# nagadomi/nunif

Measured on AMD Instinct MI355X. Metric: input MPix/s, waifu2x swin_unet 2x tiled render (tile 256) of 1080p frames, higher is better.
Workload: dtype f16; 1 GPU; waifu2x swin_unet 2x (art scale2x geometry), tile_size=256, 1080p frame, random-init weights; tile_size=256, tile_batch=45, tiles_per_frame=45, concurrent_streams=2, parallelism=frame-sharded x1

## Files before the change

### nunif_amd/csrc/swin_kernels.h

```cpp
#pragma once
#include "common.h"

namespace nunif {

struct GemmArgs {
    const f16 *a; int B, Hi, Wi, Cin;
    int Ho, Wo, stride, oy, ox, kw;
    int K;
    const f16 *w;
    const float *bias;
    int N;
    int mode;
    int act;
    float slope;
    const f16 *res;
    void *out;
    int ldo;
    int n_real;
    int ps;
    int oshift, OH, OW;
    int no_clamp;
    int lda;
    int rev;
    int nt_chunk;
    int res_H = 0, res_W = 0, res_crop = 0;
    const float *in_scale = nullptr;
};
int launch_gemm(const GemmArgs &g, hipStream_t s, const char *tag);

struct PatchUpArgs { const f16 *a, *w; const float *bias; const f16 *res; f16 *out; int B, Ho, Wo, Cq, rev; };
bool patchup_supported(const PatchUpArgs &g);
int launch_patchup(const PatchUpArgs &g, hipStream_t s);

struct PatchDownArgs { const f16 *a, *w; const float *bias; f16 *out; int B, Ho, Wo, Cin, oy, rev; int N = 192; int act = 0; float slope = 0.f; };
bool patchdown_supported(const PatchDownArgs &g);
int launch_patchdown(const PatchDownArgs &g, hipStream_t s);

struct CunetUpArgs { const f16 *a, *w; const float *bias; const f16 *res; f16 *out; const float *in_scale; int B, S, res_S, crop;
                     float slope; };
bool cunet_up_supported(const CunetUpArgs &g);
int launch_cunet_up(const CunetUpArgs &g, hipStream_t s);

struct GemmOsArgs {
    const f16 *a; long M; int lda, K;
    const f16 *w; const float *bias; int N;
    int act;
    const f16 *res;
    f16 *out; int ldo;
    float2 *stats_out;
    const float2 *stats_in; int stats_parts; const float *wsum; float ln_eps;
};
bool gemm_os_supported(long M, int N, int K);
bool gemm_os_consumes_stats(long M, int N, int K);
int launch_gemm_os(const GemmOsArgs &g, hipStream_t s, const char *tag);

struct DaMlpArgs {
    f16 *t; long M;
    const f16 *w1; const float *b1, *ws1;
    const f16 *w2c; const float *b2;
    const float2 *stats_in; float2 *stats_out; float ln_eps;
    void *partial; unsigned *flags;
};
bool da_mlp_supported(int D, int hidden);

struct CunetHeadArgs { const f16 *a, *w; const float *bias; float *out32; const float *add32; int B, Hi, Wi, Ho, Wo, addH, addW, add_crop, clamp01; };
bool cunet_head_supported(const CunetHeadArgs &g);
int launch_cunet_head(const CunetHeadArgs &g, hipStream_t s);

constexpr int kVdaGnBlocks = 256;
int launch_vda_groupnorm(const f16 *x, const float *gamma, const float *beta, f16 *y, float2 *part, int frames, int P, int C, float eps, hipStream_t s);
int launch_vda_layernorm(const f16 *x, const float *gamma, const float *beta, f16 *y, long T, int C, float eps, hipStream_t s);
int launch_vda_geglu(const f16 *h, f16 *out, long T, int I, hipStream_t s);
struct VdaTattnArgs { const f16 *qkv; f16 *kc, *vc; const float *pq, *pk, *pv; f16 *att; int P, C, hd, start, idx; };
int launch_vda_tattn(const VdaTattnArgs &g, hipStream_t s);
long da_mlp_partial_bytes(long M);
long da_mlp_flag_count(long M);
int launch_da_mlp(const DaMlpArgs &a, hipStream_t s);

struct Stem1Args {
    const float *x;
    int frame_mode, H, W, wb, istep, pad_t, pad_l, tile_begin;
    int B, T;
    const float *w;
    const float *bias;
    int C1, C1P;
    f16 *out;
    float slope;
};
int launch_stem1(const Stem1Args &a, hipStream_t s);

struct StemFusedArgs {
    const float *x;
    int frame_mode, H, W, wb, istep, pad_t, pad_l, tile_begin;
    int B, T;
    const f16 *w1;
    const f16 *w2;
    const float *b2;
    f16 *out;
    float slope;
    int rev;
    int C1, C, crop;
};
bool stem_fused_supported(int C1, int C);
int launch_stem_fused(const StemFusedArgs &a, hipStream_t s);

int proj_mlp_stream_frags(int C);
struct TailToImage { const f16 *w; const float *bias; float *out; int H, W, ps, n_real; };
struct WinMap { int on, H, W, shift; const int *pixmap; };
int launch_winmap_build(int *pixmap, int B, int H, int W, int shift, hipStream_t s);
int launch_proj_mlp(const f16 *att, f16 *x, const f16 *wstream, const float *bp, const float *b0, const float *b3,
                    long M, int C, hipStream_t s, const TailToImage *to_image = nullptr, int rev = 0,
                    const WinMap *wm = nullptr, int gelu32 = 0);

int swin_block96_tail_frags();
int swin_block96_btab_floats();
int launch_swin_block96(f16 *x, const f16 *wqkv, const float *bqkv, const float *btab, const f16 *wtail, const float *bp,
                        const float *b0, const float *b3, int B, int H, int W, int shift, hipStream_t s,
// ... 62 lines not shown
```

### nunif_amd/csrc/swin_patchdown.hip

```cpp
#include <algorithm>
#include <cstdlib>

#include "swin_kernels.h"

namespace nunif {

#define MFMA_16x16x32(a, b, c) __builtin_amdgcn_mfma_f32_16x16x32_f16((a), (b), (c), 0, 0, 0)

namespace {
constexpr int kWaves = 8;
constexpr int kMF = 2;

__device__ __forceinline__ void dma16(const void *src, unsigned lds_byte_addr) {
    asm volatile("s_mov_b32 m0, %1\n\ts_nop 0\n\tglobal_load_lds_dwordx4 %0, off" ::"v"(src), "s"(lds_byte_addr) : "memory");
}
}

template <int CIN, int kKS, int kNT, bool LRELU>
__global__ void __launch_bounds__(kWaves * 64) patchdown_kernel(PatchDownArgs g) {
    static_assert(CIN == 64 || CIN == 96 || CIN == 192, "Cin");
    constexpr int kWBytes = kNT * kKS * 1024;
    extern __shared__ __attribute__((aligned(1024))) unsigned char smem_pd[];
    const f16x8 *wres = reinterpret_cast<const f16x8 *>(smem_pd);
    const float4 *bres = reinterpret_cast<const float4 *>(smem_pd + kWBytes);
    const int tid = threadIdx.x, lane = tid & 63, r16 = lane & 15, grp = lane >> 4;
    const int wave = __builtin_amdgcn_readfirstlane(tid >> 6);
    {
        const unsigned char *src = reinterpret_cast<const unsigned char *>(g.w) + lane * 16;
        const unsigned lds0 = (unsigned)reinterpret_cast<size_t>(smem_pd);
#pragma unroll
        for (int u = 0; u < kWBytes / 1024 / kWaves; ++u) {
            const int i = wave + kWaves * u;
            dma16(src + (size_t)i * 1024, lds0 + i * 1024);
        }
        if (tid < kNT * 4) reinterpret_cast<float4 *>(smem_pd + kWBytes)[tid] = reinterpret_cast<const float4 *>(g.bias)[tid];
    }
    const unsigned Wo = (unsigned)g.Wo, Ho = (unsigned)g.Ho, Wi = 2 * Wo, Hi = 2 * Ho;
    const unsigned M = (unsigned)g.B * Ho * Wo;
    const unsigned n_groups = (M + kMF * 16 - 1) / (kMF * 16);
    const unsigned step = gridDim.x * kWaves;
    unsigned gi = blockIdx.x * kWaves + wave;
    const bool any = gi < n_groups;
    const int prc = pair_run_channel(grp);

    struct Grp { unsigned in[kMF], out[kMF]; };
    auto coords = [&](unsigned gidx, Grp &c) {
        const unsigned gg = g.rev ? n_groups - 1 - gidx : gidx;
#pragma unroll
        for (int f = 0; f < kMF; ++f) {
            unsigned m = gg * (kMF * 16) + f * 16 + r16;
            m = m < M ? m : M - 1;
            const unsigned t = m / Wo, x = m - t * Wo;
            const unsigned b = t / Ho, y = t - b * Ho;
            c.in[f] = (((b * Hi + 2 * y + (unsigned)g.oy) * Wi + 2 * x) * CIN + grp * 8) * 2;
            c.out[f] = (m * (kNT * 16) + prc) * 2;
        }
    };
    auto ks_off = [&](int ks) -> unsigned {
        const int k0 = ks * 32, tap = k0 / CIN, c0 = k0 % CIN;
        const int dy = tap / 2, dx = tap % 2;
        return (unsigned)((dy * Wi + dx) * CIN + c0) * 2;
    };
    auto load_frag = [&](const Grp &c, int f, int ks) -> f16x8 {
        const unsigned char *base = reinterpret_cast<const unsigned char *>(g.a) + (size_t)ks_off(ks);
        return *reinterpret_cast<const f16x8 *>(base + (size_t)c.in[f]);
    };

    Grp cur, nxt;
    f16x8 xf[kMF][kKS];
    coords(any ? gi : 0, cur);
#pragma unroll
    for (int ks = 0; ks < kKS; ++ks) {
#pragma unroll
        for (int f = 0; f < kMF; ++f) xf[f][ks] = load_frag(cur, f, ks);
    }
    asm volatile("s_waitcnt vmcnt(0)" ::: "memory");
#pragma unroll
    for (int ks = 0; ks < kKS; ++ks) {
#pragma unroll
        for (int f = 0; f < kMF; ++f) asm volatile("" : "+v"(xf[f][ks]));
    }
    __syncthreads();
    if (!any) return;

    while (true) {
        const unsigned gn = gi + step;
        const bool has_next = gn < n_groups;
        coords(has_next ? gn : gi, nxt);
        int lofs = lane;
        asm volatile("" : "+v"(lofs));
        f32x4 acc[kNT][kMF];
#pragma unroll
        for (int nt = 0; nt < kNT; ++nt) {
            const float4 bv = bres[nt * 4 + (lofs >> 4)];
#pragma unroll
            for (int f = 0; f < kMF; ++f) acc[nt][f] = (f32x4){bv.x, bv.y, bv.z, bv.w};
        }
#pragma unroll
        for (int ks = 0; ks < kKS; ++ks) {
#pragma unroll
            for (int nt = 0; nt < kNT; ++nt) {
                const f16x8 wv = wres[(nt * kKS + ks) * 64 + lofs];
#pragma unroll
                for (int f = 0; f < kMF; ++f) acc[nt][f] = MFMA_16x16x32(wv, xf[f][ks], acc[nt][f]);
            }
#pragma unroll
            for (int f = 0; f < kMF; ++f) xf[f][ks] = load_frag(nxt, f, ks);
            __builtin_amdgcn_sched_barrier(0);
        }
        unsigned char *obase = reinterpret_cast<unsigned char *>(g.out);
#pragma unroll
        for (int p = 0; p < kNT / 2; ++p) {
#pragma unroll
            for (int f = 0; f < kMF; ++f) {
                f32x4 a0 = acc[2 * p][f], a1 = acc[2 * p + 1][f];
                if constexpr (LRELU) {
#pragma unroll
                    for (int r = 0; r < 4; ++r) {
                        a0[r] = a0[r] >= 0.f ? a0[r] : a0[r] * g.slope;
                        a1[r] = a1[r] >= 0.f ? a1[r] : a1[r] * g.slope;
                    }
                }
                const f16x8 ov = pair_to_run((f16x4){(f16)a0[0], (f16)a0[1], (f16)a0[2], (f16)a0[3]},
                                             (f16x4){(f16)a1[0], (f16)a1[1], (f16)a1[2], (f16)a1[3]});
                *reinterpret_cast<f16x8 *>(obase + (size_t)cur.out[f] + p * 64) = ov;
            }
        }
        if (!has_next) break;
        cur = nxt;
        gi = gn;
    }
}

bool patchdown_supported(const PatchDownArgs &g) {
    if (const char *e = getenv("NUNIF_PATCHDOWN")) if (atoi(e) == 0) return false;
    const long M = (long)g.B * g.Ho * g.Wo;
    const bool shape = (g.Cin == 96 && g.N == 192 && g.oy == 0) || (g.Cin == 192 && g.N == 192 && (g.oy == 0 || g.oy == 1)) ||
                       (g.Cin == 64 && g.N == 64 && g.oy == 0);
    const bool act_ok = g.Cin == 64 ? g.act == 2 : g.act == 0;
    return shape && M > 0 && 4 * M * g.Cin * 2 < (1L << 32) && M * g.N * 2 < (1L << 32) && act_ok;
}

template <int CIN, int KS, int NT, bool LRELU>
static int launch_pd(const PatchDownArgs &g, hipStream_t s, const char *name, int wgs_per_cu) {
    constexpr int smem = NT * KS * 1024 + NT * 16 * 4;
    static_assert(smem <= 160 * 1024, "LDS");
    const long M = (long)g.B * g.Ho * g.Wo;
    static bool configured = false;
    static int cus = 256;
    if (!configured) {
        NUNIF_HIP_CHECK(hipFuncSetAttribute((const void *)patchdown_kernel<CIN, KS, NT, LRELU>, hipFuncAttributeMaxDynamicSharedMemorySize, smem));
        int dev = 0;
        NUNIF_HIP_CHECK(hipGetDevice(&dev));
        NUNIF_HIP_CHECK(hipDeviceGetAttribute(&cus, hipDeviceAttributeMultiprocessorCount, dev));
        configured = true;
    }
    const long groups = (M + kMF * 16 - 1) / (kMF * 16);
    const unsigned grid = (unsigned)std::max<long>(1, std::min<long>((groups + kWaves - 1) / kWaves, (long)cus * wgs_per_cu));
    ProfScope ps(name, s, 2.0 * (double)M * (KS * 32.0) * (NT * 16.0), (double)M * (KS * 32.0 + NT * 16.0) * 2.0);
    patchdown_kernel<CIN, KS, NT, LRELU><<<grid, kWaves * 64, smem, s>>>(g);
    NUNIF_LAUNCH_CHECK();
    return NUNIF_HIP_OK;
}

int launch_patchdown(const PatchDownArgs &g, hipStream_t s) {
    NUNIF_REQUIRE(g.a && g.w && g.bias && g.out && patchdown_supported(g), "patchdown: bad argument");
    if (g.Cin == 96) return launch_pd<96, 12, 12, false>(g, s, "patchdown_kernel<96>", 1);
    if (g.Cin == 192) return launch_pd<192, 12, 12, false>(g, s, "patchdown_kernel<192>", 1);
    return launch_pd<64, 8, 4, true>(g, s, "patchdown_kernel<64>", 2);
}

}
```

### nunif_amd/csrc/swin_stem.hip

```cpp
#include <algorithm>
#include <cstdlib>
#include <cstring>

#include "swin_kernels.h"

namespace nunif {

#define MFMA_16x16x32(a, b, c) __builtin_amdgcn_mfma_f32_16x16x32_f16((a), (b), (c), 0, 0, 0)

namespace {
constexpr int kTile = 16;
constexpr int kWaves = 8;

template <int C1, int C, int CROP, int ROWS>
struct StemGeom {
    static constexpr int kTH = kWaves * ROWS;
    static constexpr int kS1H = kTH + 2, kS1W = kTile + 2;
    static constexpr int kInH = kTH + 4, kInW = kTile + 4;
    static constexpr int kInElems = 3 * kInH * kInW;
    static constexpr int kInBytes = (kInElems + 8) * 2;
    static constexpr int kPix = C1 * 2 + 16;
    static constexpr int kKS2 = (9 * C1 + 31) / 32;
    static constexpr int kNT1 = C1 / 16, kNT2 = C / 16;
    static constexpr int kW2Bytes = kKS2 * kNT2 * 1024, kW1Bytes = kNT1 * 1024, kS1Bytes = kS1H * kS1W * kPix;
// ... 90 lines not shown
    __syncthreads();

#pragma unroll 1
    for (int t = blockIdx.x; t < n_tiles; t += gridDim.x) {
        const int tm = tmap(t);
        const int txt = tm % ntx, t2 = tm / ntx;
        const int tyt = t2 % nty, b = t2 / nty;
        f16x8 w1f[kNT1];
#pragma unroll
        for (int nt = 0; nt < kNT1; ++nt) w1f[nt] = w1g[nt * 64 + lane];
#pragma unroll
        for (int i = 0; i < kNIn; ++i) {
            const int e = tid + kWaves * 64 * i;
            if (e < kInElems) inl[e] = (f16)pin[i];
        }
        __syncthreads();
#pragma unroll
        for (int i = 0; i < kR1; ++i) {
            const int mt = wave + kWaves * i;
            if (mt * 16 < kS1H * kS1W) {
                const int p = min(mt * 16 + r16, kS1H * kS1W - 1);
                const int py = p / kS1W, px = p - py * kS1W;
                const int pb = py * kInW + px;
                f16x8 bfrag;
#pragma unroll
                for (int j = 0; j < 8; ++j) bfrag[j] = inl[ioff[j] + ((cmask >> j) & 1u ? 0 : pb)];
                const bool wr = mt * 16 + r16 < kS1H * kS1W;
#pragma unroll
                for (int nt = 0; nt < kNT1; ++nt) {
                    f32x4 acc = {0.f, 0.f, 0.f, 0.f};
                    acc = MFMA_16x16x32(w1f[nt], bfrag, acc);
                    f16x4 o;
#pragma unroll
                    for (int q = 0; q < 4; ++q) o[q] = (f16)(acc[q] >= 0.f ? acc[q] : acc[q] * a.slope);
                    if (wr) *reinterpret_cast<f16x4 *>(s1l + p * kPix + (16 * nt + 4 * grp) * 2) = o;
                }
            }
        }
        __syncthreads();
        if (t + (int)gridDim.x < n_tiles) fetch_in(tmap(t + gridDim.x), pin);
        f32x4 acc[kNT2][ROWS];
#pragma unroll
        for (int nt = 0; nt < kNT2; ++nt) {
            const f32x4 bb = *reinterpret_cast<const f32x4 *>(b2l + 16 * nt + 4 * grp);
#pragma unroll
            for (int f = 0; f < ROWS; ++f) acc[nt][f] = bb;
        }
        const unsigned char *bp0 = s1l + ((ROWS * wave) * kS1W + r16) * kPix;
#pragma unroll
        for (int ks = 0; ks < kKS2; ++ks) {
            f16x8 bf[ROWS];
#pragma unroll
            for (int f = 0; f < ROWS; ++f) bf[f] = *reinterpret_cast<const f16x8 *>(bp0 + f * (kS1W * kPix) + koff[ks]);
#pragma unroll
            for (int nt = 0; nt < kNT2; ++nt) {
                const f16x8 w = w2l[(ks * kNT2 + nt) * 64 + lane];
#pragma unroll
                for (int f = 0; f < ROWS; ++f) acc[nt][f] = MFMA_16x16x32(w, bf[f], acc[nt][f]);
            }
        }
        const int ox = kTile * txt + r16;
#pragma unroll
        for (int f = 0; f < ROWS; ++f) {
            const int oy = kTH * tyt + ROWS * wave + f;
            const bool ok = oy < S && ox < S;
            f16 *op = a.out + (((long)b * S + min(oy, S - 1)) * S + min(ox, S - 1)) * kC + pair_run_channel(grp);
#pragma unroll
            for (int p = 0; p < kNT2 / 2; ++p) {
                f16x4 oa, ob;
#pragma unroll
                for (int q = 0; q < 4; ++q) {
                    const float u = acc[2 * p][f][q], v = acc[2 * p + 1][f][q];
                    oa[q] = (f16)(u >= 0.f ? u : u * a.slope);
                    ob[q] = (f16)(v >= 0.f ? v : v * a.slope);
                }
                const f16x8 o = pair_to_run(oa, ob);
                if (ok) *reinterpret_cast<f16x8 *>(op + 32 * p) = o;
            }
        }
        __syncthreads();
    }
}

bool stem_fused_supported(int C1, int C) { return (C1 == 48 && C == 96) || (C1 == 32 && C == 64); }

template <int C1, int C, int CROP, int ROWS>
static int launch_stem_t(const StemFusedArgs &a, hipStream_t s, const char *name) {
    typedef StemGeom<C1, C, CROP, ROWS> G;
    const int S = a.T - 4 - 2 * CROP;
    NUNIF_REQUIRE(S > 0, "stem: tile size %d too small", a.T);
    const int ntx = (S + kTile - 1) / kTile, nty = (S + G::kTH - 1) / G::kTH;
    const long n_tiles = (long)a.B * ntx * nty;
    if (n_tiles == 0) return NUNIF_HIP_OK;
    const double px = (double)a.B * S * S;
    ProfScope ps(name, s, 2.0 * px * (27.0 * C1 + 9.0 * C1 * C), px * (12.0 + C * 2.0));
    static bool configured = false;
    if (!configured) {
        NUNIF_HIP_CHECK(hipFuncSetAttribute((const void *)stem_fused_kernel<C1, C, CROP, ROWS>, hipFuncAttributeMaxDynamicSharedMemorySize,
                                            G::kSmem));
        configured = true;
    }
    const unsigned grid = (unsigned)std::min<long>(n_tiles, G::kSmem <= 80 * 1024 ? 512 : 256);
    stem_fused_kernel<C1, C, CROP, ROWS><<<grid, kWaves * 64, G::kSmem, s>>>(a);
    NUNIF_LAUNCH_CHECK();
    return NUNIF_HIP_OK;
}

int launch_stem_fused(const StemFusedArgs &a, hipStream_t s) {
    static const int rows = getenv("NUNIF_STEM_ROWS") && atoi(getenv("NUNIF_STEM_ROWS")) == 2 ? 2 : 3;
    static const int rows_c = getenv("NUNIF_STEM_ROWS_CUNET") && atoi(getenv("NUNIF_STEM_ROWS_CUNET")) == 3 ? 3 : 2;
    if (a.C1 == 32 && a.C == 64 && a.crop == 0)
        return rows_c == 3 ? launch_stem_t<32, 64, 0, 3>(a, s, "stem_fused_kernel<32,64>") : launch_stem_t<32, 64, 0, 2>(a, s, "stem_fused_kernel<32,64>");
    NUNIF_REQUIRE((a.C1 == 48 || a.C1 == 0) && (a.C == 96 || a.C == 0), "stem: C1=%d C=%d unsupported", a.C1, a.C);
    return rows == 3 ? launch_stem_t<48, 96, 6, 3>(a, s, "stem_fused_kernel") : launch_stem_t<48, 96, 6, 2>(a, s, "stem_fused_kernel");
}

}
```

### nunif_amd/csrc/swin_unet.cpp

```cpp
#include <algorithm>
#include <cmath>
#include <cstdlib>
#include <cstring>
#include <map>
#include <string>
#include <vector>

#include "swin_kernels.h"

namespace nunif {

int launch_stitch(const float *tile_out, float *y, const nunif_tile_grid *g, int C, hipStream_t s, int y0 = 0, int rows = -1,
                  int compact = 0);

namespace {

struct HostTensor { const float *data; std::vector<int64_t> shape; int64_t numel; };

struct Linear {
    f16 *w = nullptr;
    float *bias = nullptr;
    int N = 0, n_real = 0, K = 0;
};

// ... 233 lines not shown
            const float *pd = pw->data;
            std::vector<f16> hpc = pack_a_fragments(dim, dim, [=](int n, int k) { return pd[(size_t)n * dim + k]; }, true);
            const int KS = dim / 32, NT = dim / 16, SH = 2 * dim / 32;
            std::vector<f16> stream((size_t)swin_block96_tail_frags() * 512, (f16)0.0f);
            size_t fi = 0;
            auto put = [&](const std::vector<f16> &src, int frag) {
                std::copy(src.begin() + (size_t)frag * 512, src.begin() + (size_t)(frag + 1) * 512, stream.begin() + fi * 512);
                ++fi;
            };
            for (int sx = 0; sx < KS; ++sx)
                for (int ks = 0; ks < KS; ++ks) { put(hpc, (2 * sx) * KS + ks); put(hpc, (2 * sx + 1) * KS + ks); }
            for (int sx = 0; sx < SH; ++sx) {
                for (int ks = 0; ks < KS; ++ks) { put(h0, (2 * sx) * KS + ks); put(h0, (2 * sx + 1) * KS + ks); }
                for (int nt = 0; nt < NT; ++nt) put(h3, nt * SH + sx);
            }
            NUNIF_REQUIRE((int)fi == swin_block96_tail_frags(), "internal: block96 stream has %zu fragments", fi);
            if ((rc = upload(h, stream, &bl.b96_tail))) return rc;
            const int stride = swin_block96_btab_floats() / heads;
            std::vector<float> rt((size_t)heads * stride, -1000.0f);
            for (int hh = 0; hh < heads; ++hh) {
                for (int i2 = 0; i2 < 121; ++i2) rt[(size_t)hh * stride + i2] = tab->data[(size_t)(120 - i2) * heads + hh] * 1.4426950408889634f;
                rt[(size_t)hh * stride + 121] = rt[(size_t)hh * stride + 122] = rt[(size_t)hh * stride + 123] = 0.0f;
            }
            if ((rc = upload(h, rt, &bl.b96_btab))) return rc;
        }
        std::vector<float> bias((size_t)heads * 36 * 48);
        for (int hh = 0; hh < heads; ++hh)
            for (int q = 0; q < 36; ++q)
                for (int k = 0; k < 48; ++k) {
                    float v = -1.0e30f;
                    if (k < 36) {
                        const int idx = (q / 6 - k / 6 + 5) * 11 + (q % 6 - k % 6 + 5);
                        v = tab->data[(size_t)idx * heads + hh];
                    }
                    bias[((size_t)hh * 36 + q) * 48 + k] = v;
                }
        if ((rc = upload(h, bias, &bl.attn_bias))) return rc;
        std::vector<float> btab32((size_t)heads * 36 * 52, 0.0f);
        for (int hh = 0; hh < heads; ++hh)
            for (int q = 0; q < 36; ++q)
                for (int k = 0; k < 48; ++k) {
                    const int key = k < 32 ? k : (((k - 32) & 3) == 0 ? 32 + ((k - 32) >> 2) : -1);
                    btab32[((size_t)hh * 36 + q) * 52 + k] =
                        key >= 0 ? bias[((size_t)hh * 36 + q) * 48 + key] * 1.4426950408889634f : -1000.0f;
                }
        if (kQkvBiasFragMajor) {
            std::vector<float> frag((size_t)heads * kQkvBiasFloatsPerHead, 0.0f);
            for (int hh = 0; hh < heads; ++hh)
                for (int qt = 0; qt < 3; ++qt)
                    for (int kt = 0; kt < 3; ++kt)
                        for (int lane = 0; lane < 64; ++lane) {
                            const int r16 = lane & 15, grp = lane >> 4;
                            const int q = qt < 2 ? 16 * qt + r16 : ((r16 & 3) == 0 ? 32 + (r16 >> 2) : 35);
                            for (int j = 0; j < 4; ++j)
                                frag[((((size_t)hh * 3 + qt) * 3 + kt) * 64 + lane) * 4 + j] =
                                    btab32[((size_t)hh * 36 + q) * 52 + 16 * kt + 4 * grp + j];
                        }
            btab32.swap(frag);
        }
        if ((rc = upload(h, btab32, &bl.attn_btab32))) return rc;
    }
    return NUNIF_HIP_OK;
}

int run_gemm(const Linear &L, const f16 *a, int B, int Hi, int Wi, int Cin, int Ho, int Wo, int stride, int oy,
             int ox, int kw, int mode, int act, float slope, const f16 *res, void *out, int ldo, int ps,
             hipStream_t s, const char *tag, int rev = 0) {
    GemmArgs g;
    g.a = a; g.B = B; g.Hi = Hi; g.Wi = Wi; g.Cin = Cin;
    g.Ho = Ho; g.Wo = Wo; g.stride = stride; g.oy = oy; g.ox = ox; g.kw = kw;
    g.K = L.K; g.w = L.w; g.bias = L.bias; g.N = L.N;
    g.mode = mode; g.act = act; g.slope = slope; g.res = res; g.out = out; g.ldo = ldo;
    g.n_real = L.n_real; g.ps = ps; g.oshift = 0; g.OH = 0; g.OW = 0; g.no_clamp = 0; g.lda = 0; g.nt_chunk = 0; g.rev = rev;
    return launch_gemm(g, s, tag);
}

int run_patchup(const Linear &L, const f16 *a, int B, int H, int W, int Cq, f16 *skip, hipStream_t s, const char *tag, int rev) {
    PatchUpArgs p = {a, L.w, L.bias, skip, skip, B, H, W, Cq, rev};
    if (L.K == 192 && L.n_real == 4 * Cq && patchup_supported(p)) return launch_patchup(p, s);
    return run_gemm(L, a, B, H, W, L.K, H, W, 1, 0, 0, 1, 1, 0, 0.f, skip, skip, Cq, 1, s, tag, rev);
}

int run_patchdown(const Linear &L, const f16 *a, int B, int Ho, int Wo, int Cin, int oy, f16 *out, hipStream_t s, const char *tag,
                  int rev) {
    PatchDownArgs p;
    p.a = a; p.w = L.w; p.bias = L.bias; p.out = out; p.B = B; p.Ho = Ho; p.Wo = Wo; p.Cin = Cin; p.oy = oy; p.rev = rev;
    if (L.K == 384 && L.n_real == 192 && patchdown_supported(p)) return launch_patchdown(p, s);
    return run_gemm(L, a, B, 2 * Ho, 2 * Wo, Cin, Ho, Wo, 2, oy, 0, 2, 0, 0, 0.f, nullptr, out, L.n_real, 1, s, tag, rev);
}

int run_linear(const Linear &L, const f16 *a, int B, int H, int W, int act, const f16 *res, f16 *out,
               hipStream_t s, const char *tag, int rev = 0) {
    return run_gemm(L, a, B, H, W, L.K, H, W, 1, 0, 0, 1, 0, act, 0.f, res, out, L.n_real, 1, s, tag, rev);
}

int tap(nunif_swin_unet *h, const std::string &name, const void *src, size_t bytes, hipStream_t s) {
    if (!h->taps_on) return NUNIF_HIP_OK;
    void *p = nullptr;
    NUNIF_HIP_CHECK(hipMalloc(&p, bytes));
    NUNIF_HIP_CHECK(hipMemcpyAsync(p, src, bytes, hipMemcpyDeviceToDevice, s));
    h->taps.push_back({name, p, bytes});
    return NUNIF_HIP_OK;
}

static int next_dir(nunif_swin_unet *h) {
    const int d = h->dir;
    h->dir ^= 1;
    return d;
}

int run_stage(nunif_swin_unet *h, std::vector<Block> &blocks, f16 *x, int B, int S, int dim, hipStream_t s,
              const char *name, const TailToImage *to_image = nullptr) {
    f16 *qkv = (f16 *)h->qkv.p, *att = (f16 *)h->att.p;
    const size_t tok = (size_t)B * S * S;
    int rc;
    for (size_t i = 0; i < blocks.size(); ++i) {
        Block &bl = blocks[i];
        const int shift = (i % 2 == 1) ? 3 : 0;
        const std::string tn = std::string(name) + ".b" + std::to_string(i);
        if (!bl.fast) {
            f16 *hid = (f16 *)h->hid.p;
            const f16 *xin = x;
            if (bl.norm1) {
                if ((rc = launch_layernorm_nobias(x, hid, bl.norm1, (long)tok, dim, s))) return rc;
                xin = hid;
            }
            if ((rc = run_linear(bl.qkv, xin, B, S, S, 0, nullptr, qkv, s, "gemm_qkv", next_dir(h)))) return rc;
            if ((rc = tap(h, tn + ".qkv", qkv, tok * 3 * dim * 2, s))) return rc;
            if ((rc = launch_window_attn(qkv, att, bl.attn_bias, B, S, S, h->heads, dim / h->heads, shift, s))) return rc;
            if ((rc = tap(h, tn + ".attn", att, tok * dim * 2, s))) return rc;
            if ((rc = run_linear(bl.proj, att, B, S, S, 0, x, x, s, "gemm_proj", next_dir(h)))) return rc;
            xin = x;
            if (bl.norm2) {
                if ((rc = launch_layernorm_nobias(x, att, bl.norm2, (long)tok, dim, s))) return rc;
                xin = att;
            }
            if ((rc = run_linear(bl.mlp0p, xin, B, S, S, 1, nullptr, hid, s, "gemm_mlp0", next_dir(h)))) return rc;
            if ((rc = run_linear(bl.mlp3p, hid, B, S, S, 0, x, x, s, "gemm_mlp3", next_dir(h)))) return rc;
            if ((rc = tap(h, tn + ".out", x, tok * dim * 2, s))) return rc;
            continue;
        }
        const bool last_blk = i + 1 == blocks.size();
        if (dim == 96 && bl.b96_tail && h->block96 && !h->taps_on) {
            if ((rc = launch_swin_block96(x, bl.qkv_res, bl.qkv_rbias, bl.b96_btab, bl.b96_tail, bl.proj.bias, bl.mlp0.bias,
                                          bl.mlp3.bias, B, S, S, shift, s, last_blk ? to_image : nullptr, next_dir(h))))
                return rc;
            if (last_blk && to_image) break;
            continue;
        }
        const bool att_wm = dim == 96 && h->att_wm && !h->taps_on && 96L * (long)tok < (1L << 31);
        if ((rc = launch_qkv_attn_r(x, att, bl.qkv_res, bl.qkv_rbias, bl.attn_btab32, B, S, S, dim, h->heads, shift, s, next_dir(h),
                                    att_wm ? 1 : 0)))
            return rc;
        if ((rc = tap(h, tn + ".attn", att, tok * dim * 2, s))) return rc;
        const bool last = i + 1 == blocks.size();
        if (dim == 192) {
            if ((rc = launch_proj_mlp_ws(att, x, bl.tail_ws, bl.proj.bias, bl.mlp0.bias, bl.mlp3.bias, (long)tok, s, next_dir(h), h->gelu32)))
                return rc;
        } else {
            const int eff_shift = S <= 6 ? 0 : shift;
            WinMap wmap = {att_wm ? 1 : 0, S, S, eff_shift, nullptr};
            if (att_wm) {
                if (h->winmap_S != S || B > h->winmap_B) {
                    for (int k = 0; k < 2; ++k) {
                        if ((rc = h->winmap[k].ensure(tok * sizeof(int)))) return rc;
                        if ((rc = launch_winmap_build((int *)h->winmap[k].p, B, S, S, k ? 3 : 0, s))) return rc;
                    }
                    h->winmap_B = B; h->winmap_S = S;
                }
                wmap.pixmap = (const int *)h->winmap[eff_shift ? 1 : 0].p;
            }
            if ((rc = launch_proj_mlp(att, x, bl.tail_stream, bl.proj.bias, bl.mlp0.bias, bl.mlp3.bias, (long)tok, dim, s,
                                      last ? to_image : nullptr, next_dir(h), &wmap, h->gelu32)))
                return rc;
        }
        if (last && to_image) break;
        if ((rc = tap(h, tn + ".out", x, tok * dim * 2, s))) return rc;
    }
    return NUNIF_HIP_OK;
}

int ensure_workspace(nunif_swin_unet *h, int B, int T) {
    const size_t S = T - 16, S2 = S / 2, S4 = S / 4, C = h->C;
    const size_t t1 = (size_t)B * S * S, t2 = (size_t)B * S2 * S2, t3 = (size_t)B * S4 * S4;
    const size_t top = h->top_dim;
    int rc;
    if ((rc = h->s1.ensure((size_t)B * (T - 14) * (T - 14) * h->C1P * 2))) return rc;
    if ((rc = h->f1.ensure(t1 * C * 2))) return rc;
    if ((rc = h->f2.ensure(t2 * 2 * C * 2))) return rc;
    if ((rc = h->f3.ensure(t3 * 2 * C * 2))) return rc;
    if (h->has_proj2 && (rc = h->g1.ensure(t1 * top * 2))) return rc;
    const size_t qkv_elems = std::max(t1 * 3 * std::max(C, top), t2 * 6 * C);
    if ((rc = h->qkv.ensure(qkv_elems * 2))) return rc;
    if ((rc = h->att.ensure(std::max(t1 * std::max(C, top), t2 * 2 * C) * 2))) return rc;
    if ((rc = h->hid.ensure(std::max(t1 * 2 * std::max(C, top), t2 * 4 * C) * 2))) return rc;
    return NUNIF_HIP_OK;
}

int forward_impl(nunif_swin_unet *h, const float *x, const float *frame, const nunif_tile_grid *grid,
                 int tile_begin, float *z, int B, int T, hipStream_t s) {
    const int S = T - 16, C = h->C;
    NUNIF_REQUIRE(T > 16 && S % 12 == 0 && S % 16 == 0, "tile_size %d is not valid for swin_unet", T);
    int rc;
    if ((rc = ensure_workspace(h, B, T))) return rc;
    f16 *s1 = (f16 *)h->s1.p, *f1 = (f16 *)h->f1.p, *f2 = (f16 *)h->f2.p, *f3 = (f16 *)h->f3.p;

    if (h->stemf_w2 && stem_fused_supported(h->C1, (int)C)) {
        StemFusedArgs sf;
        memset(&sf, 0, sizeof(sf));
        if (frame) {
            sf.x = frame; sf.frame_mode = 1; sf.H = grid->x_h; sf.W = grid->x_w; sf.wb = grid->w_blocks;
            sf.istep = grid->input_tile_step; sf.pad_t = grid->pad_t; sf.pad_l = grid->pad_l; sf.tile_begin = tile_begin;
        } else {
            sf.x = x;
        }
        sf.B = B; sf.T = T; sf.w1 = h->stemf_w1; sf.w2 = h->stemf_w2; sf.b2 = h->stem2.bias; sf.out = f1; sf.slope = 0.1f;
        h->dir = 1;
        if ((rc = launch_stem_fused(sf, s))) return rc;
        goto stem_done;
    }
    Stem1Args a1;
    memset(&a1, 0, sizeof(a1));
    if (frame) {
        a1.x = frame; a1.frame_mode = 1; a1.H = grid->x_h; a1.W = grid->x_w; a1.wb = grid->w_blocks;
        a1.istep = grid->input_tile_step; a1.pad_t = grid->pad_t; a1.pad_l = grid->pad_l; a1.tile_begin = tile_begin;
    } else {
        a1.x = x;
    }
    a1.B = B; a1.T = T; a1.w = h->stem1_w; a1.bias = h->stem1_b; a1.C1 = h->C1; a1.C1P = h->C1P; a1.out = s1;
    a1.slope = 0.1f;
    h->dir = 1;
    if ((rc = launch_stem1(a1, s))) return rc;
    if ((rc = run_gemm(h->stem2, s1, B, T - 14, T - 14, h->C1P, S, S, 1, 0, 0, 3, 0, 2, 0.1f, nullptr, f1, C, 1, s,
                              "gemm_stem2", next_dir(h))))
        return rc;
stem_done:
    if ((rc = tap(h, "stem", f1, (size_t)B * S * S * C * 2, s))) return rc;
    if ((rc = run_stage(h, h->swin[0], f1, B, S, C, s, "swin1"))) return rc;
    if ((rc = run_patchdown(h->down1, f1, B, S / 2, S / 2, C, 0, f2, s, "gemm_down1", next_dir(h)))) return rc;
    if ((rc = tap(h, "down1", f2, (size_t)B * (S / 2) * (S / 2) * 2 * C * 2, s))) return rc;
    if ((rc = run_stage(h, h->swin[1], f2, B, S / 2, 2 * C, s, "swin2"))) return rc;
    if (h->down2_split) {
        if ((rc = run_patchdown(h->down2, f2, B, S / 4, S / 4, 2 * C, 0, f3, s, "gemm_down2", next_dir(h)))) return rc;
    } else if ((rc = run_gemm(h->down2, f2, B, S / 2, S / 2, 2 * C, S / 4, S / 4, 2, 0, 0, 2, 0, 0, 0.f, nullptr, f3,
                              2 * C, 1, s, "gemm_down2", next_dir(h))))
        return rc;
    if (h->down2_split && (rc = run_gemm(h->down2b, f2, B, S / 2, S / 2, 2 * C, S / 4, S / 4, 2, 1, 0, 2, 0, 0, 0.f, f3, f3,
                                         2 * C, 1, s, "gemm_down2b", next_dir(h))))
        return rc;
    if ((rc = tap(h, "down2", f3, (size_t)B * (S / 4) * (S / 4) * 2 * C * 2, s))) return rc;
    if ((rc = run_stage(h, h->swin[2], f3, B, S / 4, 2 * C, s, "swin3"))) return rc;
    if ((rc = run_patchup(h->up2, f3, B, S / 4, S / 4, 2 * C, f2, s, "gemm_up2", next_dir(h)))) return rc;
    if ((rc = tap(h, "up2", f2, (size_t)B * (S / 2) * (S / 2) * 2 * C * 2, s))) return rc;
    if ((rc = run_stage(h, h->swin[3], f2, B, S / 2, 2 * C, s, "swin4"))) return rc;
    f16 *top = f1;
    if (h->has_proj2) {
        top = (f16 *)h->g1.p;
        if ((rc = run_linear(h->proj2, f1, B, S, S, 0, nullptr, top, s, "gemm_proj2", next_dir(h)))) return rc;
    }
    if ((rc = run_patchup(h->up1, f2, B, S / 2, S / 2, h->top_dim, top, s, "gemm_up1", next_dir(h)))) return rc;
    if ((rc = tap(h, "up1", top, (size_t)B * S * S * h->top_dim * 2, s))) return rc;
    if (h->top_dim == 96 && h->swin[4].back().fast && h->to_image_chained && !h->taps_on) {
        TailToImage ti;
        ti.w = h->to_image_chained; ti.bias = h->to_image.bias; ti.out = z; ti.H = S; ti.W = S; ti.ps = h->scale_factor;
        ti.n_real = h->to_image.n_real;
        return run_stage(h, h->swin[4], top, B, S, h->top_dim, s, "swin5", &ti);
    }
    if ((rc = run_stage(h, h->swin[4], top, B, S, h->top_dim, s, "swin5"))) return rc;
    if (h->scale_factor == 8) {
        f16 *pre = (f16 *)h->att.p;
        if ((rc = run_gemm(h->to_image_pre, top, B, S, S, h->top_dim, S, S, 1, 0, 0, 1, 0, 2, 0.2f, nullptr, pre, 192, 1, s,
                           "gemm_to_image_pre", next_dir(h))))
            return rc;
        top = pre;
    }
    if ((rc = run_gemm(h->to_image, top, B, S, S, h->top_dim, S, S, 1, 0, 0, 1, 2, 0, 0.f, nullptr, z, 0,
                       h->scale_factor, s, "gemm_to_image", next_dir(h))))
        return rc;
    return NUNIF_HIP_OK;
}

}
}

extern "C" int nunif_hip_swin_unet_create(const nunif_tensor_desc *tensors, int32_t n_tensors,
                                          int32_t scale_factor, nunif_swin_unet **handle) {
    NUNIF_REQUIRE(tensors && handle && n_tensors > 0, "swin_unet_create: NULL argument");
    NUNIF_REQUIRE(scale_factor == 1 || scale_factor == 2 || scale_factor == 4 || scale_factor == 8,
                  "swin_unet_create: scale_factor %d unsupported (1, 2, 4, 8)", scale_factor);
    TensorMap m;
    for (int i = 0; i < n_tensors; ++i) {
        HostTensor t;
        t.data = tensors[i].data;
        t.numel = 1;
        for (int d = 0; d < tensors[i].ndim; ++d) {
            t.shape.push_back(tensors[i].shape[d]);
            t.numel *= tensors[i].shape[d];
        }
        m[tensors[i].name] = t;
    }
    nunif_swin_unet *h = new nunif_swin_unet();
    (void)hipGetDevice(&h->device);
    if (const char *v = getenv("NUNIF_BLOCK96")) h->block96 = atoi(v);
    if (const char *v = getenv("NUNIF_ATT_WM")) h->att_wm = atoi(v);
    h->gelu32 = scale_factor == 1;
    if (const char *v = getenv("NUNIF_SWIN_GELU32")) h->gelu32 = atoi(v);
    h->scale_factor = scale_factor;
    const std::string P = "unet.";
    int rc = NUNIF_HIP_OK;
    do {
        const HostTensor *w0, *b0, *w2, *b2;
        if ((rc = find(m, P + "patch.0.weight", &w0)) || (rc = find(m, P + "patch.0.bias", &b0)) ||
            (rc = find(m, P + "patch.2.weight", &w2)) || (rc = find(m, P + "patch.2.bias", &b2)))
            break;
        if (w2->shape.size() != 4 || w0->shape.size() != 4 || w0->shape[1] != 3) {
            set_error("patch conv: unexpected shape"); rc = NUNIF_HIP_EINVAL; break;
        }
        const int C = (int)w2->shape[0];
        const int C1 = (int)w0->shape[0];
        if (C % 96 != 0 || C1 * 2 != C) { set_error("base_dim %d unsupported", C); rc = NUNIF_HIP_EUNSUPPORTED; break; }
        h->C = C; h->heads = C / 16; h->C1 = C1; h->C1P = (C1 + 31) / 32 * 32;
        h->has_proj2 = scale_factor >= 4;
        h->top_dim = h->has_proj2 ? 2 * C : C;
        {
            std::vector<float> w(w0->data, w0->data + w0->numel), b(b0->data, b0->data + b0->numel);
            if ((rc = upload(h, w, &h->stem1_w)) || (rc = upload(h, b, &h->stem1_b))) break;
        }
        {
            const float *wd = w2->data;
            const int C1P = h->C1P;
            rc = make_linear(h, C, 9 * C1P, [=](int n, int k) {
// ... 206 lines not shown
```

Before: 328.7 MPix/s.

## Route down2b through patchdown kernel with fused residual accumulation; add pipelined stem kernel

Adds an accumulate mode to the specialized patchdown kernel, which reads the existing output, adds bias and residual in the epilogue, and prefetches residual rows during the last k-steps. The second half of the split down2 projection now uses this kernel instead of the generic GEMM with a residual. It also adds an opt-in persistent stem kernel that software-pipelines conv1 of the next tile under conv2 of the current one, gated behind an environment variable that is off by default. The cost is an extra template instantiation, more register pressure in the accumulate path, and a reliance on res aliasing out.

```diff
diff --git a/nunif_amd/csrc/swin_kernels.h b/nunif_amd/csrc/swin_kernels.h
--- a/nunif_amd/csrc/swin_kernels.h
+++ b/nunif_amd/csrc/swin_kernels.h
@@ -32,7 +32,8 @@
 bool patchup_supported(const PatchUpArgs &g);
 int launch_patchup(const PatchUpArgs &g, hipStream_t s);
 
-struct PatchDownArgs { const f16 *a, *w; const float *bias; f16 *out; int B, Ho, Wo, Cin, oy, rev; int N = 192; int act = 0; float slope = 0.f; };
+struct PatchDownArgs { const f16 *a, *w; const float *bias; f16 *out; int B, Ho, Wo, Cin, oy, rev; int N = 192; int act = 0; float slope = 0.f;
+                       const f16 *res = nullptr; };
 bool patchdown_supported(const PatchDownArgs &g);
 int launch_patchdown(const PatchDownArgs &g, hipStream_t s);
 
diff --git a/nunif_amd/csrc/swin_patchdown.hip b/nunif_amd/csrc/swin_patchdown.hip
--- a/nunif_amd/csrc/swin_patchdown.hip
+++ b/nunif_amd/csrc/swin_patchdown.hip
@@ -16,7 +16,7 @@
 }
 }
 
-template <int CIN, int kKS, int kNT, bool LRELU>
+template <int CIN, int kKS, int kNT, bool LRELU, bool ACC>
 __global__ void __launch_bounds__(kWaves * 64) patchdown_kernel(PatchDownArgs g) {
     static_assert(CIN == 64 || CIN == 96 || CIN == 192, "Cin");
     constexpr int kWBytes = kNT * kKS * 1024;
@@ -92,10 +92,12 @@
         f32x4 acc[kNT][kMF];
 #pragma unroll
         for (int nt = 0; nt < kNT; ++nt) {
-            const float4 bv = bres[nt * 4 + (lofs >> 4)];
+            const float4 bv = ACC ? float4{0.f, 0.f, 0.f, 0.f} : bres[nt * 4 + (lofs >> 4)];
 #pragma unroll
             for (int f = 0; f < kMF; ++f) acc[nt][f] = (f32x4){bv.x, bv.y, bv.z, bv.w};
         }
+        const unsigned char *rbase = reinterpret_cast<const unsigned char *>(g.out);
+        f16x8 rres[kMF];
 #pragma unroll
         for (int ks = 0; ks < kKS; ++ks) {
 #pragma unroll
@@ -104,6 +106,12 @@
 #pragma unroll
                 for (int f = 0; f < kMF; ++f) acc[nt][f] = MFMA_16x16x32(wv, xf[f][ks], acc[nt][f]);
             }
+            if constexpr (ACC) {
+                if (ks == kKS - 2) {
+#pragma unroll
+                    for (int f = 0; f < kMF; ++f) rres[f] = *reinterpret_cast<const f16x8 *>(rbase + (size_t)cur.out[f]);
+                }
+            }
 #pragma unroll
             for (int f = 0; f < kMF; ++f) xf[f][ks] = load_frag(nxt, f, ks);
             __builtin_amdgcn_sched_barrier(0);
@@ -111,6 +119,23 @@
         unsigned char *obase = reinterpret_cast<unsigned char *>(g.out);
 #pragma unroll
         for (int p = 0; p < kNT / 2; ++p) {
+            if constexpr (ACC) {
+                const float4 b0 = bres[(2 * p) * 4 + (lofs >> 4)], b1 = bres[(2 * p + 1) * 4 + (lofs >> 4)];
+#pragma unroll
+                for (int f = 0; f < kMF; ++f) {
+                    f32x4 &a0 = acc[2 * p][f], &a1 = acc[2 * p + 1][f];
+                    f16x4 ra, rb;
+                    run_to_pair(rres[f], ra, rb);
+                    a0[0] += b0.x; a0[1] += b0.y; a0[2] += b0.z; a0[3] += b0.w;
+                    a1[0] += b1.x; a1[1] += b1.y; a1[2] += b1.z; a1[3] += b1.w;
+#pragma unroll
+                    for (int r = 0; r < 4; ++r) { a0[r] += (float)ra[r]; a1[r] += (float)rb[r]; }
+                }
+                if (p + 1 < kNT / 2) {
+#pragma unroll
+                    for (int f = 0; f < kMF; ++f) rres[f] = *reinterpret_cast<const f16x8 *>(rbase + (size_t)cur.out[f] + (p + 1) * 64);
+                }
+            }
 #pragma unroll
             for (int f = 0; f < kMF; ++f) {
                 f32x4 a0 = acc[2 * p][f], a1 = acc[2 * p + 1][f];
@@ -138,10 +163,14 @@
     const bool shape = (g.Cin == 96 && g.N == 192 && g.oy == 0) || (g.Cin == 192 && g.N == 192 && (g.oy == 0 || g.oy == 1)) ||
                        (g.Cin == 64 && g.N == 64 && g.oy == 0);
     const bool act_ok = g.Cin == 64 ? g.act == 2 : g.act == 0;
+    if (g.res) {
+        if (!(g.Cin == 192 && g.res == g.out)) return false;
+        if (const char *e = getenv("NUNIF_PATCHDOWN_ACC")) if (atoi(e) == 0) return false;
+    }
     return shape && M > 0 && 4 * M * g.Cin * 2 < (1L << 32) && M * g.N * 2 < (1L << 32) && act_ok;
 }
 
-template <int CIN, int KS, int NT, bool LRELU>
+template <int CIN, int KS, int NT, bool LRELU, bool ACC = false>
 static int launch_pd(const PatchDownArgs &g, hipStream_t s, const char *name, int wgs_per_cu) {
     constexpr int smem = NT * KS * 1024 + NT * 16 * 4;
     static_assert(smem <= 160 * 1024, "LDS");
@@ -149,7 +178,7 @@
     static bool configured = false;
     static int cus = 256;
     if (!configured) {
-        NUNIF_HIP_CHECK(hipFuncSetAttribute((const void *)patchdown_kernel<CIN, KS, NT, LRELU>, hipFuncAttributeMaxDynamicSharedMemorySize, smem));
+        NUNIF_HIP_CHECK(hipFuncSetAttribute((const void *)patchdown_kernel<CIN, KS, NT, LRELU, ACC>, hipFuncAttributeMaxDynamicSharedMemorySize, smem));
         int dev = 0;
         NUNIF_HIP_CHECK(hipGetDevice(&dev));
         NUNIF_HIP_CHECK(hipDeviceGetAttribute(&cus, hipDeviceAttributeMultiprocessorCount, dev));
@@ -157,8 +186,8 @@
     }
     const long groups = (M + kMF * 16 - 1) / (kMF * 16);
     const unsigned grid = (unsigned)std::max<long>(1, std::min<long>((groups + kWaves - 1) / kWaves, (long)cus * wgs_per_cu));
-    ProfScope ps(name, s, 2.0 * (double)M * (KS * 32.0) * (NT * 16.0), (double)M * (KS * 32.0 + NT * 16.0) * 2.0);
-    patchdown_kernel<CIN, KS, NT, LRELU><<<grid, kWaves * 64, smem, s>>>(g);
+    ProfScope ps(name, s, 2.0 * (double)M * (KS * 32.0) * (NT * 16.0), (double)M * (KS * 32.0 + (ACC ? 2 : 1) * NT * 16.0) * 2.0);
+    patchdown_kernel<CIN, KS, NT, LRELU, ACC><<<grid, kWaves * 64, smem, s>>>(g);
     NUNIF_LAUNCH_CHECK();
     return NUNIF_HIP_OK;
 }
@@ -166,6 +195,7 @@
 int launch_patchdown(const PatchDownArgs &g, hipStream_t s) {
     NUNIF_REQUIRE(g.a && g.w && g.bias && g.out && patchdown_supported(g), "patchdown: bad argument");
     if (g.Cin == 96) return launch_pd<96, 12, 12, false>(g, s, "patchdown_kernel<96>", 1);
+    if (g.Cin == 192 && g.res) return launch_pd<192, 12, 12, false, true>(g, s, "patchdown_kernel<192,acc>", 1);
     if (g.Cin == 192) return launch_pd<192, 12, 12, false>(g, s, "patchdown_kernel<192>", 1);
     return launch_pd<64, 8, 4, true>(g, s, "patchdown_kernel<64>", 2);
 }
diff --git a/nunif_amd/csrc/swin_stem.hip b/nunif_amd/csrc/swin_stem.hip
--- a/nunif_amd/csrc/swin_stem.hip
+++ b/nunif_amd/csrc/swin_stem.hip
@@ -196,6 +196,236 @@
     }
 }
 
+namespace {
+template <int C1, int C>
+struct StemPipeGeom {
+    static constexpr int kTH = kTile;
+    static constexpr int kS1H = kTH + 2, kS1W = kTile + 2, kInH = kTH + 4, kInW = kTile + 4;
+    static constexpr int kInElems = 3 * kInH * kInW;
+    static constexpr int kInBytes = (kInElems + 8) * 2;
+    static constexpr int kPix = C1 * 2 + 16;
+    static constexpr int kKS2 = (9 * C1 + 31) / 32;
+    static constexpr int kNT1 = C1 / 16, kNT2 = C / 16;
+    static constexpr int kW2Bytes = kKS2 * kNT2 * 1024, kS1Bytes = kS1H * kS1W * kPix;
+    static constexpr int kSmem = kW2Bytes + 2 * kS1Bytes + 2 * kInBytes + C * 4;
+    static_assert(C1 % 16 == 0 && C % 32 == 0 && (kPix / 16) % 2 == 1 && kInBytes % 16 == 0 && kS1Bytes % 16 == 0, "stem geometry");
+    static_assert(kSmem <= 160 * 1024, "LDS");
+};
+}
+
+template <int C1, int C, int CROP>
+__global__ void __launch_bounds__(kWaves * 64) stem_pipe_kernel(StemFusedArgs a) {
+    typedef StemPipeGeom<C1, C> G;
+    constexpr int kPix = G::kPix, kKS2 = G::kKS2, kNT1 = G::kNT1, kNT2 = G::kNT2, kW2Bytes = G::kW2Bytes, kS1Bytes = G::kS1Bytes;
+    constexpr int kTH = G::kTH, kS1H = G::kS1H, kS1W = G::kS1W, kInH = G::kInH, kInW = G::kInW, kInElems = G::kInElems;
+    constexpr int kInBytes = G::kInBytes, kRows = 2;
+    constexpr int kNIn = (kInElems + kWaves * 64 - 1) / (kWaves * 64);
+    constexpr int kNPix1 = kS1H * kS1W;
+    constexpr int kR1 = ((kNPix1 + 15) / 16 + kWaves - 1) / kWaves;
+    static_assert(4 * kR1 <= kKS2 - 1, "a conv1 round takes three k-steps of conv2, the input write the one behind them");
+    extern __shared__ __attribute__((aligned(16))) unsigned char smem_s[];
+    const f16x8 *w2l = reinterpret_cast<const f16x8 *>(smem_s);
+    unsigned char *s1l = smem_s + kW2Bytes;
+    unsigned char *inl = s1l + 2 * kS1Bytes;
+    float *b2l = reinterpret_cast<float *>(inl + 2 * kInBytes);
+
+    const int tid = threadIdx.x;
+    const int lane = tid & 63;
+    const int wave = __builtin_amdgcn_readfirstlane(tid >> 6);
+    const int r16 = lane & 15;
+    const int grp = lane >> 4;
+
+    {
+        f16x8 *dst = reinterpret_cast<f16x8 *>(smem_s);
+        const f16x8 *src2 = reinterpret_cast<const f16x8 *>(a.w2);
+        for (int i = tid; i < kW2Bytes / 16; i += kWaves * 64) dst[i] = src2[i];
+        if (tid < C) b2l[tid] = a.b2[tid];
+        if (tid < 2) {
+            f16 *ib = reinterpret_cast<f16 *>(inl + tid * kInBytes);
+            ib[kInElems] = (f16)1.0f; ib[kInElems + 1] = (f16)0.0f;
+        }
+    }
+    int ioff[8];
+    unsigned cmask = 0;
+#pragma unroll
+    for (int j = 0; j < 8; ++j) {
+        const int k = 8 * grp + j;
+        const int ci = k / 9, r = k - 9 * ci;
+        ioff[j] = k < 27 ? ci * (kInH * kInW) + (r / 3) * kInW + (r % 3) : (k == 27 ? kInElems : kInElems + 1);
+        if (k >= 27) cmask |= 1u << j;
+    }
+    int koff[kKS2];
+#pragma unroll
+    for (int ks = 0; ks < kKS2; ++ks) {
+        int k0 = 32 * ks + 8 * grp;
+        if (k0 >= 9 * C1) k0 = 0;
+        const int tap = k0 / C1, c = k0 - tap * C1;
+        koff[ks] = ((tap / 3) * kS1W + tap % 3) * kPix + c * 2;
+    }
+    f16x8 w1f[kNT1];
+#pragma unroll
+    for (int nt = 0; nt < kNT1; ++nt) w1f[nt] = reinterpret_cast<const f16x8 *>(a.w1)[nt * 64 + lane];
+    int pb[kR1], so[kR1];
+#pragma unroll
+    for (int i = 0; i < kR1; ++i) {
+        const int p = min((wave + kWaves * i) * 16 + r16, kNPix1 - 1);
+        const int py = p / kS1W, px = p - py * kS1W;
+        pb[i] = py * kInW + px;
+        so[i] = p * kPix + 8 * grp;
+    }
+
+    const int S = a.T - 4 - 2 * CROP;
+    const int ntx = (S + kTile - 1) / kTile, nty = (S + kTH - 1) / kTH;
+    const int n_tiles = a.B * ntx * nty;
+    const int G0 = (int)gridDim.x;
+    const int n_my = (n_tiles - 1 - (int)blockIdx.x) / G0 + 1;
+    const int t_last = (int)blockIdx.x + (n_my - 1) * G0;
+
+    auto fetch_in = [&](int t, float (&v)[kNIn]) {
+        const int txt = t % ntx, t2 = t / ntx;
+        const int tyt = t2 % nty, b = t2 / nty;
+        int fy = 0, fx = 0;
+        if (a.frame_mode) {
+            const int k = a.tile_begin + b;
+            const int ti = k / a.wb, tj = k - ti * a.wb;
+            fy = ti * a.istep - a.pad_t;
+            fx = tj * a.istep - a.pad_l;
+        }
+#pragma unroll
+        for (int i = 0; i < kNIn; ++i) {
+            const int e = tid + kWaves * 64 * i;
+            v[i] = 0.f;
+            if (e < kInElems) {
+                const int ci = e / (kInH * kInW), r = e - ci * (kInH * kInW);
+                const int iy = r / kInW, ix = r - iy * kInW;
+                const int yy = min(kTH * tyt + CROP + iy, a.T - 1), xx = min(kTile * txt + CROP + ix, a.T - 1);
+                if (a.frame_mode) {
+                    const int sy = min(max(fy + yy, 0), a.H - 1), sx = min(max(fx + xx, 0), a.W - 1);
+                    v[i] = a.x[((long)ci * a.H + sy) * a.W + sx];
+                } else {
+                    v[i] = a.x[(((long)b * 3 + ci) * a.T + yy) * a.T + xx];
+                }
+            }
+        }
+    };
+    auto store_in = [&](unsigned char *buf, const float (&v)[kNIn]) {
+#pragma unroll
+        for (int i = 0; i < kNIn; ++i) {
+            const int e = tid + kWaves * 64 * i;
+            if (e < kInElems) reinterpret_cast<f16 *>(buf)[e] = (f16)v[i];
+        }
+    };
+    auto tmap = [&](int t) { return a.rev ? n_tiles - 1 - t : t; };
+    auto c1_read = [&](const unsigned char *inb, int i) -> f16x8 {
+        const f16 *in = reinterpret_cast<const f16 *>(inb);
+        f16x8 bfrag;
+#pragma unroll
+        for (int j = 0; j < 8; ++j) bfrag[j] = in[ioff[j] + ((cmask >> j) & 1u ? 0 : pb[i])];
+        return bfrag;
+    };
+    auto c1_mfma = [&](const f16x8 &bfrag, f32x4 (&c1)[kNT1]) {
+#pragma unroll
+        for (int nt = 0; nt < kNT1; ++nt) c1[nt] = MFMA_16x16x32(w1f[nt], bfrag, ((f32x4){0.f, 0.f, 0.f, 0.f}));
+    };
+    auto c1_store = [&](unsigned char *s1b, int i, const f32x4 (&c1)[kNT1]) {
+#pragma unroll
+        for (int nt = 0; nt < kNT1; ++nt) {
+            f16x4 o;
+#pragma unroll
+            for (int q = 0; q < 4; ++q) o[q] = (f16)(c1[nt][q] >= 0.f ? c1[nt][q] : c1[nt][q] * a.slope);
+            *reinterpret_cast<f16x4 *>(s1b + so[i] + 32 * nt) = o;
+        }
+    };
+
+    float pin[kNIn];
+    {
+        float pin1[kNIn];
+        fetch_in(tmap((int)blockIdx.x), pin);
+        fetch_in(tmap(min((int)blockIdx.x + G0, t_last)), pin1);
+        store_in(inl, pin);
+        store_in(inl + kInBytes, pin1);
+    }
+    __syncthreads();
+#pragma unroll
+    for (int i = 0; i < kR1; ++i) {
+        f32x4 c1[kNT1];
+        c1_mfma(c1_read(inl, i), c1);
+        c1_store(s1l, i, c1);
+    }
+    __syncthreads();
+
+#pragma unroll 1
+    for (int j = 0; j < n_my; ++j) {
+        const int t = (int)blockIdx.x + j * G0;
+        const int par = j & 1;
+        const unsigned char *s1r = s1l + par * kS1Bytes;
+        unsigned char *s1w = s1l + (par ^ 1) * kS1Bytes;
+        const unsigned char *inr = inl + (par ^ 1) * kInBytes;
+        unsigned char *inw = inl + par * kInBytes;
+        fetch_in(tmap(min(t + 2 * G0, t_last)), pin);
+
+        f32x4 acc[kNT2][kRows];
+#pragma unroll
+        for (int nt = 0; nt < kNT2; ++nt) {
+            const f32x4 bb = *reinterpret_cast<const f32x4 *>(b2l + 16 * nt + 4 * grp);
+#pragma unroll
+            for (int f = 0; f < kRows; ++f) acc[nt][f] = bb;
+        }
+        const unsigned char *bp0 = s1r + ((kRows * wave) * kS1W + r16) * kPix;
+        f16x8 bf[2][kRows], wf[2][kNT2];
+        auto load_ks = [&](int ks) {
+#pragma unroll
+            for (int f = 0; f < kRows; ++f) bf[ks & 1][f] = *reinterpret_cast<const f16x8 *>(bp0 + f * (kS1W * kPix) + koff[ks]);
+#pragma unroll
+            for (int nt = 0; nt < kNT2; ++nt) wf[ks & 1][nt] = w2l[(ks * kNT2 + nt) * 64 + lane];
+        };
+        load_ks(0);
+        f16x8 c1b;
+        f32x4 c1[kNT1];
+#pragma unroll
+        for (int ks = 0; ks < kKS2; ++ks) {
+            if (ks + 1 < kKS2) load_ks(ks + 1);
+#pragma unroll
+            for (int nt = 0; nt < kNT2; ++nt) {
+#pragma unroll
+                for (int f = 0; f < kRows; ++f) acc[nt][f] = MFMA_16x16x32(wf[ks & 1][nt], bf[ks & 1][f], acc[nt][f]);
+            }
+            if (ks < 4 * kR1) {
+                if (ks % 4 == 0) c1b = c1_read(inr, ks / 4);
+                if (ks % 4 == 1) c1_mfma(c1b, c1);
+                if (ks % 4 == 2) c1_store(s1w, ks / 4, c1);
+            } else if (ks == 4 * kR1) {
+                store_in(inw, pin);
+            }
+            __builtin_amdgcn_sched_barrier(0);
+        }
+        __syncthreads();
+
+        const int tm = tmap(t);
+        const int txt = tm % ntx, t2 = tm / ntx;
+        const int tyt = t2 % nty, b = t2 / nty;
+        const int ox = kTile * txt + r16;
+#pragma unroll
+        for (int f = 0; f < kRows; ++f) {
+            const int oy = kTH * tyt + kRows * wave + f;
+            const bool ok = oy < S && ox < S;
+            f16 *op = a.out + (((long)b * S + min(oy, S - 1)) * S + min(ox, S - 1)) * C + pair_run_channel(grp);
+#pragma unroll
+            for (int p = 0; p < kNT2 / 2; ++p) {
+                f16x4 oa, ob;
+#pragma unroll
+                for (int q = 0; q < 4; ++q) {
+                    const float u = acc[2 * p][f][q], v = acc[2 * p + 1][f][q];
+                    oa[q] = (f16)(u >= 0.f ? u : u * a.slope);
+                    ob[q] = (f16)(v >= 0.f ? v : v * a.slope);
+                }
+                const f16x8 o = pair_to_run(oa, ob);
+                if (ok) *reinterpret_cast<f16x8 *>(op + 32 * p) = o;
+            }
+        }
+    }
+}
+
 bool stem_fused_supported(int C1, int C) { return (C1 == 48 && C == 96) || (C1 == 32 && C == 64); }
 
 template <int C1, int C, int CROP, int ROWS>
@@ -220,12 +450,42 @@
     return NUNIF_HIP_OK;
 }
 
+static long stem_grid_cap() {
+    const char *e = getenv("NUNIF_STEM_GRID");
+    const long v = e ? atol(e) : 0;
+    return v > 0 ? v : (1L << 30);
+}
+
+template <int C1, int C, int CROP>
+static int launch_stem_pipe_t(const StemFusedArgs &a, hipStream_t s, const char *name) {
+    typedef StemPipeGeom<C1, C> G;
+    const int S = a.T - 4 - 2 * CROP;
+    NUNIF_REQUIRE(S > 0, "stem: tile size %d too small", a.T);
+    const int ntx = (S + kTile - 1) / kTile, nty = (S + G::kTH - 1) / G::kTH;
+    const long n_tiles = (long)a.B * ntx * nty;
+    if (n_tiles == 0) return NUNIF_HIP_OK;
+    NUNIF_REQUIRE(n_tiles < (1L << 30), "stem: %ld tiles", n_tiles);
+    const double px = (double)a.B * S * S;
+    ProfScope ps(name, s, 2.0 * px * (27.0 * C1 + 9.0 * C1 * C), px * (12.0 + C * 2.0));
+    static bool configured = false;
+    if (!configured) {
+        NUNIF_HIP_CHECK(hipFuncSetAttribute((const void *)stem_pipe_kernel<C1, C, CROP>, hipFuncAttributeMaxDynamicSharedMemorySize, G::kSmem));
+        configured = true;
+    }
+    const unsigned grid = (unsigned)std::min<long>(std::min<long>(n_tiles, 256), stem_grid_cap());
+    stem_pipe_kernel<C1, C, CROP><<<grid, kWaves * 64, G::kSmem, s>>>(a);
+    NUNIF_LAUNCH_CHECK();
+    return NUNIF_HIP_OK;
+}
+
 int launch_stem_fused(const StemFusedArgs &a, hipStream_t s) {
     static const int rows = getenv("NUNIF_STEM_ROWS") && atoi(getenv("NUNIF_STEM_ROWS")) == 2 ? 2 : 3;
     static const int rows_c = getenv("NUNIF_STEM_ROWS_CUNET") && atoi(getenv("NUNIF_STEM_ROWS_CUNET")) == 3 ? 3 : 2;
     if (a.C1 == 32 && a.C == 64 && a.crop == 0)
         return rows_c == 3 ? launch_stem_t<32, 64, 0, 3>(a, s, "stem_fused_kernel<32,64>") : launch_stem_t<32, 64, 0, 2>(a, s, "stem_fused_kernel<32,64>");
     NUNIF_REQUIRE((a.C1 == 48 || a.C1 == 0) && (a.C == 96 || a.C == 0), "stem: C1=%d C=%d unsupported", a.C1, a.C);
+    const char *pipe = getenv("NUNIF_STEM_PIPE");
+    if (pipe && atoi(pipe) != 0) return launch_stem_pipe_t<48, 96, 6>(a, s, "stem_pipe_kernel");
     return rows == 3 ? launch_stem_t<48, 96, 6, 3>(a, s, "stem_fused_kernel") : launch_stem_t<48, 96, 6, 2>(a, s, "stem_fused_kernel");
 }
 
diff --git a/nunif_amd/csrc/swin_unet.cpp b/nunif_amd/csrc/swin_unet.cpp
--- a/nunif_amd/csrc/swin_unet.cpp
+++ b/nunif_amd/csrc/swin_unet.cpp
@@ -339,11 +339,11 @@
 }
 
 int run_patchdown(const Linear &L, const f16 *a, int B, int Ho, int Wo, int Cin, int oy, f16 *out, hipStream_t s, const char *tag,
-                  int rev) {
+                  int rev, const f16 *res = nullptr) {
     PatchDownArgs p;
-    p.a = a; p.w = L.w; p.bias = L.bias; p.out = out; p.B = B; p.Ho = Ho; p.Wo = Wo; p.Cin = Cin; p.oy = oy; p.rev = rev;
+    p.a = a; p.w = L.w; p.bias = L.bias; p.out = out; p.B = B; p.Ho = Ho; p.Wo = Wo; p.Cin = Cin; p.oy = oy; p.rev = rev; p.res = res;
     if (L.K == 384 && L.n_real == 192 && patchdown_supported(p)) return launch_patchdown(p, s);
-    return run_gemm(L, a, B, 2 * Ho, 2 * Wo, Cin, Ho, Wo, 2, oy, 0, 2, 0, 0, 0.f, nullptr, out, L.n_real, 1, s, tag, rev);
+    return run_gemm(L, a, B, 2 * Ho, 2 * Wo, Cin, Ho, Wo, 2, oy, 0, 2, 0, 0, 0.f, res, out, L.n_real, 1, s, tag, rev);
 }
 
 int run_linear(const Linear &L, const f16 *a, int B, int H, int W, int act, const f16 *res, f16 *out,
@@ -502,8 +502,7 @@
     } else if ((rc = run_gemm(h->down2, f2, B, S / 2, S / 2, 2 * C, S / 4, S / 4, 2, 0, 0, 2, 0, 0, 0.f, nullptr, f3,
                               2 * C, 1, s, "gemm_down2", next_dir(h))))
         return rc;
-    if (h->down2_split && (rc = run_gemm(h->down2b, f2, B, S / 2, S / 2, 2 * C, S / 4, S / 4, 2, 1, 0, 2, 0, 0, 0.f, f3, f3,
-                                         2 * C, 1, s, "gemm_down2b", next_dir(h))))
+    if (h->down2_split && (rc = run_patchdown(h->down2b, f2, B, S / 4, S / 4, 2 * C, 1, f3, s, "gemm_down2b", next_dir(h), f3)))
         return rc;
     if ((rc = tap(h, "down2", f3, (size_t)B * (S / 4) * (S / 4) * 2 * C * 2, s))) return rc;
     if ((rc = run_stage(h, h->swin[2], f3, B, S / 4, 2 * C, s, "swin3"))) return rc;
```

Result: no change. 329.4 MPix/s, median of 6 (+0.2%).
